# Roman-HLIS-Cosmology-PIT/romanimpreprocess

Measured on AMD Instinct MI355X. Metric: SCA ramps/sec (4096x4096x8grp full L1->L2 chain), higher is better.
Workload: dtype f32

## Files before the change

include/romanhip.h:

```cpp
#ifndef ROMANHIP_H
#define ROMANHIP_H

#include <stdint.h>

#ifdef __cplusplus
extern "C" {
#endif

#define RIP_VERSION 100
#define RIP_TIMING_BUILD_FLAG 1000000
#define RIP_MAX_GROUPS 64
#define RIP_CHANNEL_WIDTH 128

typedef struct rip_ctx rip_ctx;

typedef enum { RIP_OK = 0, RIP_EINVAL = -1, RIP_ENOMEM = -2, RIP_EHIP = -3, RIP_ESTATE = -4 } rip_status;
typedef enum { RIP_F32 = 0, RIP_F64 = 1, RIP_U16 = 2, RIP_F16 = 3 } rip_dtype;
typedef enum { RIP_HOST = 0, RIP_DEVICE = 1 } rip_location;
typedef enum { RIP_INPUTS_STREAM_ORDERED = 0, RIP_INPUTS_COMPLETE = 1 } rip_inputs_ready;

enum {
    RIP_STAGE_REFPIX = 1 << 0,
    RIP_STAGE_BIAS = 1 << 1,
    RIP_STAGE_LIN = 1 << 2,
// ... 174 lines not shown

int rip_stage_noise_1f(rip_ctx *ctx, int rows, int width, int nframes, const double *normals, uint64_t seed,
                       uint32_t stream_id, float *out);

int rip_stage_poisson_resample(rip_ctx *ctx, const float *skylevel, const void *gain, int gain_dtype, size_t n,
                               double frame_time, int ngrp, const int32_t *group_first, const int32_t *group_count,
                               const float *weights, const uint8_t *has_weights, const int8_t *endslice,
                               const double *samples, int nsamp, uint64_t seed, uint32_t layer, float *diff);


int rip_stats_l1_diff(rip_ctx *ctx, const uint16_t *cube, int ngrp, int ny, int nx, int ga, int gb, float *out);

int rip_stats_l2_pack(rip_ctx *ctx, const float *slope, const float *err_read, const float *err_poisson,
                      const uint32_t *pixeldq, int ny, int nx, int nb, const uint8_t grow[32], float *image, float *err,
                      uint8_t *good);

int rip_stats_reduce(rip_ctx *ctx, int nseeds, const float *diffs, const float *images, const float *errs, const uint8_t *good,
                     const float *ideal, int y0, int nrows, int ny, int nx, int nb, int alias_err, float *out);

int rip_profile_enable(rip_ctx *ctx, int on);
int rip_profile_read(rip_ctx *ctx, double out_ms[4], int *ncalls);

int rip_set_option(rip_ctx *ctx, const char *name, int value);
int rip_set_option_f64(rip_ctx *ctx, const char *name, double value);
int rip_get_option(rip_ctx *ctx, const char *name, int *value);
int rip_get_option_f64(rip_ctx *ctx, const char *name, double *value);
int rip_reset_options(rip_ctx *ctx);
int rip_option_info(int index, const char **name, int *def, int *lo, int *hi);

int rip_last_chain_form(rip_ctx *ctx);
int rip_last_chain_first_group(rip_ctx *ctx);
int rip_last_chain_bias_stream(rip_ctx *ctx);
int rip_last_prepass_gate(rip_ctx *ctx, int *giveups);

int rip_chain_form_for(int lin_nplanes, int ngroups, int ipc_dtype, int gain_dtype);

int rip_chain_geometry_for(int lin_nplanes, int ngroups, int ipc_dtype, int gain_dtype, int ny, int nx, int ncu, int reserve,
                           int quad_ok, int out[8]);
int rip_last_chain_geometry(rip_ctx *ctx, int out[8]);

int rip_stage_pearson(rip_ctx *ctx, size_t n, const double *I, double tilnu21, double tilnu31, double tilnu41, uint64_t seed,
                      uint32_t stream, double *draws, int32_t *types, double *params);

typedef struct rip_synth_cal {
    int32_t ny, nx, nb;
    int32_t channelwidth;
    int32_t nplanes;
    int32_t gain_dtype;
    int32_t ipc_dtype;
    int32_t amp33_valid;
    const void *gain;
    const float *read_noise;
    const float *resetnoise;
    const float *dark_slope;
    const float *dark;
    const float *lin_coefs;
    const float *smin, *smax;
    const void *ipc4d;
    const float *biascorr;
    double tbias;
    const float *amp33_med, *amp33_std;
    double m_pink, ru_pink;
    double u_pink, c_pink;
} rip_synth_cal;

int rip_synth_apportion(rip_ctx *ctx, const float *counts, int nya, int nxa, int poisson, int nreads, const double *t_reads,
// ... 83 lines not shown
```

romanimpreprocess_amd/_native.py:

```python

import contextlib
import ctypes as C
import os

import numpy as np

from . import _header

_HERE = os.path.dirname(os.path.abspath(__file__))
LIB_PATH = os.environ.get("ROMANHIP_LIB") or os.path.join(_HERE, "libromanhip.so")

with open(os.path.join(os.path.dirname(_HERE), "include", "romanhip.h")) as _f:
    HEADER = _header.parse(_f.read())
PROTOTYPES = HEADER.prototypes

globals().update(HEADER.constants)
globals().update({k[4:]: v for k, v in HEADER.constants.items() if k.startswith(("RIP_STAGE_", "RIP_BIAS_"))})

CaldirDesc = HEADER.structs["rip_caldir_desc"]
PlanDesc = HEADER.structs["rip_plan_desc"]
RampDesc = HEADER.structs["rip_ramp_desc"]
Outputs = HEADER.structs["rip_outputs"]
SynthCal = HEADER.structs["rip_synth_cal"]
CrParams = HEADER.structs["rip_cr_params"]
# ... 202 lines not shown
    def get_option_f64(self, name):
        v = C.c_double()
        self.call("rip_get_option_f64", name, C.byref(v))
        return v.value

    def reset_options(self):
        self.call("rip_reset_options")

    @contextlib.contextmanager
    def options(self, **values):
        calls = {name: ((self.get_option_f64, self.set_option_f64) if isinstance(v, float) else (self.get_option, self.set_option))
                 for name, v in values.items()}
        old = []
        try:
            for name, v in values.items():
                get, set_ = calls[name]
                before = get(name)
                set_(name, v)
                old.append((set_, name, before))
            yield self
        finally:
            for set_, name, before in reversed(old):
                set_(name, before)

    def last_chain_form(self):
        return self.call("rip_last_chain_form")

    def last_chain_first_group(self):
        return self.call("rip_last_chain_first_group")

    def last_prepass_gate(self):
        n = C.c_int(0)
        return self.call("rip_last_prepass_gate", C.byref(n)), n.value

    def caldir_first_group_safe(self, slot):
        return self.call("rip_caldir_first_group_safe", slot) == 1

    def caldir_bias_state(self, slot):
        return self.call("rip_caldir_bias_state", slot)

    def last_chain_bias_stream(self):
        return self.call("rip_last_chain_bias_stream")

    def last_chain_geometry(self):
        out = (C.c_int * 8)()
        self.call("rip_last_chain_geometry", out)
        return dict(zip(GEOMETRY_FIELDS, out))

    def profile(self, on=True):
        self.call("rip_profile_enable", bool(on))

    def profile_read(self):
        ms = (C.c_double * 4)()
        n = C.c_int(0)
        self.call("rip_profile_read", ms, C.byref(n))
        return list(ms), n.value

    @property
    def stream(self):
        return self.call("rip_stream")

    def upload_caldir(self, slot, cal, nborder=4, refout_slope=None):
        d = CaldirDesc()
        keep = []

        def P(a, dt):
# ... 76 lines not shown
```

romanimpreprocess_amd/csrc/api.hip:

```cpp
#include <limits.h>
#include <math.h>
#include <stdarg.h>
#include <stdio.h>
#include <string.h>

#include "rip_host.h"

static std::string g_create_error;

int rip_fail(rip_ctx *ctx, int code, const char *fmt, ...) {
    char buf[512];
    va_list ap;
    va_start(ap, fmt);
    vsnprintf(buf, sizeof buf, fmt, ap);
    va_end(ap);
    if (ctx)
        ctx->err = buf;
    else
        g_create_error = buf;
    return code;
}

void *rip_ws(rip_ctx *ctx, RipWs slot, size_t bytes) {
    if (ctx->ws_bytes[slot] >= bytes && ctx->ws[slot]) return ctx->ws[slot];
// ... 151 lines not shown
    if (ctx->stream2) RIP_HIP(ctx, hipStreamSynchronize(ctx->stream2));
    RIP_HIP(ctx, hipStreamSynchronize(ctx->stream));
    return RIP_OK;
}

void *rip_stream(rip_ctx *ctx) { return (void *)ctx->stream; }

void *rip_host_alloc(rip_ctx *ctx, size_t bytes) {
    void *p = nullptr;
    if (hipSetDevice(ctx->device) != hipSuccess || hipHostMalloc(&p, bytes ? bytes : 1, hipHostMallocDefault) != hipSuccess) {
        (void)rip_fail(ctx, RIP_ENOMEM, "rip_host_alloc: %zu bytes of page-locked memory", bytes);
        return nullptr;
    }
    return p;
}
void rip_host_free(rip_ctx *ctx, void *p) {
    (void)ctx;
    if (p) (void)hipHostFree(p);
}

int rip_option_info(int index, const char **name, int *def, int *lo, int *hi) {
    if (index < 0 || index >= (int)(sizeof k_options / sizeof k_options[0])) return 0;
    const RipOption &o = k_options[index];
    const auto as_int = [](double v) { return v <= INT_MIN ? INT_MIN : v >= INT_MAX ? INT_MAX : (int)v; };
    if (name) *name = o.name;
    if (def) *def = as_int(o.def);
    if (lo) *lo = as_int(o.lo);
    if (hi) *hi = as_int(o.hi);
    return o.f64 ? 2 : 1;
}

int rip_reset_options(rip_ctx *ctx) {
    for (const RipOption &o : k_options) store_option(ctx, o, o.def);
    return RIP_OK;
}

int rip_set_option(rip_ctx *ctx, const char *name, int value) { return set_option(ctx, name, false, value); }
int rip_set_option_f64(rip_ctx *ctx, const char *name, double value) { return set_option(ctx, name, true, value); }

int rip_get_option(rip_ctx *ctx, const char *name, int *value) {
    const RipOption *o = find_option(ctx, name, false);
    if (o) *value = ctx->*o->i;
    return o ? RIP_OK : RIP_EINVAL;
}
int rip_get_option_f64(rip_ctx *ctx, const char *name, double *value) {
    const RipOption *o = find_option(ctx, name, true);
    if (o) *value = ctx->*o->f64;
    return o ? RIP_OK : RIP_EINVAL;
}

int rip_chain_stamps(rip_ctx *ctx, double out[9]) {
    const size_t n = 4096 * 9;
    if (!ctx->chain_dbg_buf) {
        RIP_HIP(ctx, hipMalloc((void **)&ctx->chain_dbg_buf, n * 8));
        RIP_HIP(ctx, hipMemset(ctx->chain_dbg_buf, 0, n * 8));
        for (int i = 0; i < 9; ++i) out[i] = 0;
        return RIP_OK;
    }
    RIP_HIP(ctx, hipStreamSynchronize(ctx->stream));
    std::vector<unsigned long long> h(n);
    RIP_HIP(ctx, hipMemcpy(h.data(), ctx->chain_dbg_buf, n * 8, hipMemcpyDeviceToHost));
    for (int i = 0; i < 9; ++i) out[i] = 0;
    for (size_t k = 0; k < n; ++k) out[k % 9] += (double)h[k];
    RIP_HIP(ctx, hipMemset(ctx->chain_dbg_buf, 0, n * 8));
    return RIP_OK;
}
// ... 84 lines not shown
```

romanimpreprocess_amd/csrc/calibrate.hip:

```cpp
#include <string.h>

#include <cmath>

#include "rip_host.h"

size_t rip_host_ramp_bytes(const rip_ramp_desc &in, int ny, int nx) {
    const size_t G = in.ngrp, npix = (size_t)ny * nx;
    return al256(G * npix * (in.data_dtype == RIP_U16 ? 2 : 4)) + al256(G * ny * RIP_CW * 2) + al256(G * npix) + al256(npix * 4) +
           al256(npix * 8) + al256(G * (nx / RIP_CW) * 16) + al256(npix * 2) + al256((size_t)ny * RIP_CW * 2);
}

int rip_check_reference_read(rip_ctx *ctx, const rip_ramp_desc &in, const char *who) {
    if (!rip_ramp_is_encoded(in)) return RIP_OK;
    if (in.location == RIP_DEVICE)
        return rip_fail(ctx, RIP_EINVAL, "%s: reference_read / reference_amp33 come with host ramps only (a device caller decodes its arrays with "
                        "rip_stage_decode_reference_read and calibrates them as usual)", who);
    if (in.reference_read && in.data_dtype != RIP_U16) return rip_fail(ctx, RIP_EINVAL, "%s: reference_read needs u16 data", who);
    if (in.reference_amp33 && !in.amp33) return rip_fail(ctx, RIP_EINVAL, "%s: reference_amp33 without amp33", who);
    if (in.data_encoding_offset > (1 << 30) || in.data_encoding_offset < -(1 << 30))
        return rip_fail(ctx, RIP_EINVAL, "%s: data_encoding_offset %d (|offset| <= 2^30 supported)", who, (int)in.data_encoding_offset);
    return RIP_OK;
}

int rip_upload_host_ramp(rip_ctx *ctx, const rip_ramp_desc &in, int ny, int nx, char *w, hipStream_t st, rip_ramp_desc *dev,
// ... 287 lines not shown
        } else {
            ca.bias = c.dark_data;
            ca.bias_records = 0;
        }
        ca.planes = c.slab;
        ca.do_not_flag_first = plan->h.do_not_flag_first;
        ca.kern = c.ipc;
        ca.finish = (stages & (RIP_STAGE_DARK | RIP_STAGE_FLAT)) ? 1 : 0;
        if (stages & RIP_STAGE_DARK) {
            ca.dark_rate = 1;
            ca.dark_dq = c.has_dark_dq ? c.dark_dq : nullptr;
        }
        ca.flat = flat;
        ca.slope = o.slope;
        ca.err_read = o.err_read;
        ca.err_poisson = o.err_poisson;
        ca.pdq_out = o.pixeldq;
        ca.gdq_out = o.groupdq;
        float *cube = nullptr;
        if (out->cube) {
            cube = host ? (float *)rip_ws(ctx, RIP_WS_CUBE_B, (size_t)G * npix * 4) : out->cube;
            if (!cube) return RIP_ENOMEM;
            ca.cube_out = cube;
        }
        ca.ny = ny;
        ca.nx = nx;
        ca.nb = c.nb;
        ca.ngrp = G;
        ca.dense = plan->d_dense;
        ca.merged_dq = c.merged_plane[((flat ? 1 : 0) | ((stages & RIP_STAGE_DARK) ? 2 : 0))];
        ca.dbg = ctx->chain_dbg;
        ca.dbg_buf = ctx->chain_dbg_buf;
        ca.wg_counter = ctx->prepass_gate > 0 ? ctx->gate_words : nullptr;
        const int rc = rip_launch_chain(ctx, plan, ca, c.lin_nplanes, c.ipc_dtype, skip0);
        if (rc == 1 && skip0) return rip_fail(ctx, RIP_ESTATE, "calibrate: the fused kernel declined a launch planned without group 0");
        if (rc == 1) return RIP_OK;
        if (rc) return rc;
        ran_fused = true;
        cur = cube;
        for (int i = 0; i < 3; ++i) mark(ctx, ctx->stream);
        return RIP_OK;
    }

    int stage_kernels() {
        int rc;
        pdq_mid = d.pixeldq;
        if (do_ref || do_bias || do_lin || in->data_dtype != RIP_F32) {
            float *cubeA = (float *)rip_ws(ctx, RIP_WS_CUBE_A, (size_t)G * npix * 4 + npix * 4);
            if (!cubeA) return RIP_ENOMEM;
            uint32_t *pdq_ws = (uint32_t *)(cubeA + (size_t)G * npix);
            LinArgs la;
            memset(&la, 0, sizeof la);
            la.data = d.data;
            la.data_dtype = in->data_dtype;
            la.phi = cubeA;
            la.gdq = d.groupdq;
            la.gdq_is_attempt = 0;
            la.pdq_in = d.pixeldq;
            la.pdq_out = do_lin ? pdq_ws : nullptr;
            if (do_ref) {
                la.dark_data = c.dark_data;
                la.rowcorr = rowcorr;
                la.lines = lines;
            }
            if (do_bias) la.bias = c.bias + (size_t)(c.ngrp_bias - G) * npix;
            if (do_lin) {
// ... 112 lines not shown
```

romanimpreprocess_amd/csrc/chain2_kernel.h:

```cpp
#pragma once
#include "chain_common.h"
#include "chain2_form.h"

#if (defined(C2_DBG) || defined(CH_STAMP)) && !defined(RIP_TIMING_BUILD)
#error "C2_DBG / CH_STAMP are timing experiments: build them with -DRIP_TIMING_BUILD"
#endif
#ifdef CH_STAMP
#define C2_DRAIN()                                \
    if (a.dbg & 2048) {                           \
        __builtin_amdgcn_s_waitcnt(0);            \
    }
#else
#define C2_DRAIN()
#endif
#define C2_SYNC() __syncthreads()

__device__ __forceinline__ unsigned c2_opaque(unsigned x) {
    asm volatile("" : "+v"(x));
    return x;
}

__device__ __forceinline__ __amdgpu_buffer_rsrc_t c2_rsrc(const void *p, int records = -1) {
    return __builtin_amdgcn_make_buffer_rsrc(const_cast<void *>(p), 0, records, 0x00020000);
}
// ... 605 lines not shown
                            }
                            O12[(p0 * 3 + so) * COLS + col] = o1v;
                        }
                    }
                }
                if (GP * CO_STEP < NCO) fetch_coefs(kb2, r + 4, GP * CO_STEP, NCO, rr);
            }
            CH_T(5)
            CH_T(6)
            C2_SYNC();
            CH_T(7)
        }
    } else {
        f2 xnext[GP];
#pragma unroll
        for (int p0 = 0; p0 < GP; ++p0) xnext[p0] = f2{0.0f, 0.0f};
        const RipVariant v0 = rip_load_variant(vars, 0);
        const RipFitConst fc0 = rip_fit_const(h);
        constexpr int start = START;
        float gain_next = 1.0f;
        uint32_t dq_next = 0, qw_next[QW];
#pragma unroll
        for (int i = 0; i < QW; ++i) qw_next[i] = 0;
        int o0_r = (R0 - 5 + 3000) % 3;
        uint32_t qb_next[F::wring ? 1 : G];
#pragma unroll
        for (int g = 0; g < (F::wring ? 1 : G); ++g) qb_next[g] = 0;
        f2 kn[5];
        double kn_d[9];
#pragma unroll
        for (int i = 0; i < 5; ++i) kn[i] = f2{0.0f, 0.0f};
#pragma unroll
        for (int k = 0; k < 9; ++k) kn_d[k] = 0.0;
        for (int r = R0 - 5; r <= R0 + rows_wg; ++r, o0_r = (o0_r == 2) ? 0 : o0_r + 1) {
            const bool emit = (r >= R0) && (r < R1) && col_ok && (wcol >= 2 || c < 2) && (wcol < wl - 2 || c >= nx - 2);
            const RIP_K C2KernArgs *kf = c2_args(kargs);
            const unsigned rc_ = (unsigned)min(max(r, R0), yhi);
            const unsigned pe = rc_ * (unsigned)nx + cc1;
            const __amdgpu_buffer_rsrc_t rpl = c2_rsrc(kf->a.planes);
            const unsigned t_row = rc_ * row4;
            const unsigned t_ld = (dbg & 256) ? 0u : t_row;
            const float e_read = c2_ld_f32<SA>(rpl, cc4, (unsigned)(NP + 5) * pl4 + t_ld);
            const float e_gain = gain_next;
            const size_t t_row4 = (size_t)t_row;
            const size_t pe_row = (size_t)(rc_ * (unsigned)nx);
            const float e_dark = c2_ld_f32<SA>(rpl, cc4, (unsigned)(NP + 6) * pl4 + t_ld);
            const uint32_t e_pdq = c2_ld_u32<SA>(c2_rsrc(kf->a.pdq), cc4, t_ld);
            const float e_flat_raw = c2_ld_f32<SA>(c2_rsrc(kf->a.flat ? (const void *)kf->a.flat : (const void *)kf->a.planes), cc4, t_ld);
            const float e_flat = kf->a.flat ? e_flat_raw : 1.0f;
            float d[GE];
            f2 dpair[GP];
            uint32_t qw[QW];
#pragma unroll
            for (int i = 0; i < QW; ++i) qw[i] = 0;
            uint32_t lin_dq = 0;
            RipFitState fs;
            const bool act = emit && col_act && r >= ay0 && r < ay1;
            CH_T(0)
            C2_DRAIN()
            CH_T(1)
            f2 kF[5];
            double kFd[9];
            kF[4].y = 0.0f;
            if constexpr (KFIT) {
#pragma unroll
                for (int k = 0; k < 9; ++k) kFd[k] = kn_d[k];
#pragma unroll
                for (int i = 0; i < 5; ++i) kF[i] = kn[i];
            }
            if (emit) {
                if constexpr (KRN > 0) {
                    const int ks = r & 1;
                    if constexpr (K64) {
#pragma unroll
                        for (int k = 0; k < KRN; ++k) kFd[k] = KRd[(ks * KRN + k) * COLS + col];
                    } else {
#pragma unroll
                        for (int i = 0; i < 4; ++i) kF[i] = KR2[(ks * 4 + i) * COLS + col];
                        kF[4].x = KR1[ks * COLS + col];
                    }
                }
                const unsigned vF = k_valid(r);
#pragma unroll
                for (int i = 0; i < QW; ++i) qw[i] = qw_next[i];
                if constexpr (!F::wring) {
#pragma unroll
                    for (int i = 0; i < QW; ++i) qw[i] = 0;
#pragma unroll
                    for (int g = 0; g < G; ++g) qw[g / 4] |= (qb_next[g] & 0xffu) << (8 * (g & 3));
// ... 74 lines not shown
#pragma unroll
                            for (int b = 0; b < NBG; ++b) {
                                const f2 *ob = O12 + (p0 + b) * 3 * COLS;
                                om[b] = ob + om_ * COLS, o0[b] = ob + o0_ * COLS, op[b] = ob + op_ * COLS;
                            }
                            f2 f[NBG], oc[NBG];
                            if (all)
                                fwd_rows_batch<NBG, true>(om, o0, op, col, kF, vF, f, oc);
                            else
                                fwd_rows_batch<NBG, false>(om, o0, op, col, kF, vF, f, oc);
                            f2 o2[NBG];
#pragma unroll
                            for (int b = 0; b < NBG; ++b) o2[b] = (oc[b] + xc[b]) - f[b];
                            if (fastdiv) {
#pragma unroll
                                for (int b = 0; b < NBG; ++b) val[b] = div_rcp2(o2[b], e_gain, rgain);
                            } else {
#pragma unroll
                                for (int b = 0; b < NBG; ++b) val[b] = f2{o2[b].x / e_gain, o2[b].y / e_gain};
                            }
                        }
#pragma unroll
                        for (int b = 0; b < NBG; ++b) {
                            d[2 * (p0 + b)] = val[b].x;
                            d[2 * (p0 + b) + 1] = val[b].y;
                            dpair[p0 + b] = val[b];
                        }
                    }
                }
                if constexpr (GE > G) d[G] = 0.0f, dpair[GP - 1].y = 0.0f;
                if constexpr (SKIP0) d[0] = 0.0f, dpair[0].x = 0.0f;
                const bool unsat = ((qw[(G - 1) / 4] >> (8 * ((G - 1) & 3))) & DQ_SATURATED) == 0;
                if (!(dbg & 4))
                    fit_full_pk_a<G, rip_full_valid<G, START>(), SKIP0>(dpair, fc0, v0, kf->a.dense, e_gain, e_read, unsat && act, kf->guard, fs);
            }
            CH_T(2)
            C2_SYNC();
            CH_T(3)
            const RIP_K C2KernArgs *kg = c2_args(kargs);
            CH_T(4)
            C2_DRAIN()
            CH_T(5)
            float s = 0.0f, er = 0.0f, ep = 0.0f;
            uint32_t jmask = 0, pdq = 0;
            auto part_fb = [&]() {
                if constexpr (!SKIP0) {
                    if (kg->a.cube_out) {
#pragma unroll
                        for (int g = 0; g < G; ++g) kg->a.cube_out[(unsigned)g * npix + pe] = d[g];
                    }
                }
                uint32_t qor = 0;
#pragma unroll
                for (int i = 0; i < QW; ++i) qor |= qw[i];
                const bool anysat = (qor & 0x02020202u) != 0u;
                const bool unsat = ((qw[(G - 1) / 4] >> (8 * ((G - 1) & 3))) & DQ_SATURATED) == 0;
                if (dbg & 4) {
                    s = d[0], er = e_read, ep = e_gain;
                } else {
                    fit_full_pk_b<G>(dpair, kg->h, fc0, kg->a.dense, kg->kvals + v0.k_ofs, kg->diffs + v0.diff_ofs, unsat && act,
                                     fs, jmask);
                    s = fs.s, er = fs.er, ep = fs.ep;
                    if (__any(anysat)) {
                        uint32_t qe[G];
#pragma unroll
                        for (int g = 0; g < G; ++g) qe[g] = (qw[g / 4] >> (8 * (g & 3))) & 0xffu;
                        trunc_layers<G, G - 1, GE, SKIP0>(d, qe, kg->h, kg->vars, kg->kvals, kg->diffs, e_gain, e_read, act, kg->guard, s, er,
                                                          ep, jmask);
// ... 39 lines not shown
                part_finish();
            }
            {
                const int sn = (o0_r == 2) ? 0 : o0_r + 1;
#pragma unroll
                for (int p0 = 0; p0 < GP; ++p0) xnext[p0] = X2[(p0 * XR + sn) * COLS + col];
                dq_next = DQ[sn * COLS + col];
                if constexpr (F::wring) {
#pragma unroll
                    for (int i = 0; i < QW; ++i) qw_next[i] = QS[(sn * QW + i) * COLS + col];
                    gain_next = GN[sn * COLS + col];
                } else {
                    const unsigned yl = (unsigned)min(max((dbg & 1024) ? R0 : r + 1, ylo), yhi);
                    const __amdgpu_buffer_rsrc_t rq = c2_rsrc(kg->a.gdq);
                    unsigned o1 = yl * (row4 >> 2);
#pragma unroll
                    for (int g = 0; g < G; ++g) {
                        qb_next[g] = c2_ld_u8(rq, cc1, o1);
                        o1 += npix;
                    }
                    gain_next = c2_ld_f32(c2_rsrc(kg->a.planes), cc4, (unsigned)(NP + 4) * pl4 + yl * row4);
                }
            }
            if constexpr (KFIT) {
                if constexpr (K64)
                    (void)load_k(kg->a.kern, (dbg & 1024) ? R0 : r + 1, true, kn_d, C2Int<KRN>{});
                else
                    (void)load_k(kg->a.kern, (dbg & 1024) ? R0 : r + 1, true, kn, C2Int<0>{});
            }
            CH_T(6)
            C2_SYNC();
            CH_T(7)
        }
    }
#ifdef CH_STAMP
    if ((tid & 63) == 0 && a.dbg_buf) {
        unsigned long long *o = a.dbg_buf + ((size_t)blockIdx.x * (F::threads / 64) + (tid >> 6)) * 9;
        for (int i = 0; i < 9; ++i) o[i] += st_[i];
    }
#endif
}

template <int NP, int G, int START, typename KT, bool SKIP0 = false, bool BIAS = true>
static int launch_chain2_s(rip_ctx *ctx, const RipPlan *plan, const ChainArgs &a) {
    using F = C2Form<G + (G & 1), sizeof(KT) == 8>;
    const size_t lds = F::lds_bytes;
    if (a.nb < 2) return 1;
    ChainArgs ag = a;
    const long grid = c2_form_geometry<F>(ag, ctx->ncu, ctx->chain_reserve, ctx->chain_quad, ctx->last_geo);
    static bool lds_set[64] = {};
    if (lds > 48 * 1024 && !lds_set[ctx->device & 63]) {
        RIP_HIP(ctx, hipFuncSetAttribute(reinterpret_cast<const void *>(chain2_kernel<NP, G, START, KT, SKIP0, BIAS>),
                                         hipFuncAttributeMaxDynamicSharedMemorySize, (int)lds));
        lds_set[ctx->device & 63] = true;
    }
    hipLaunchKernelGGL((chain2_kernel<NP, G, START, KT, SKIP0, BIAS>), dim3((unsigned)grid), dim3(F::threads), lds, ctx->stream, ag,
                       reinterpret_cast<const RipPlanHeader *>(plan->dev), plan->d_variants, plan->d_k, plan->d_diffs,
                       ctx->guard_band);
    RIP_HIP(ctx, hipGetLastError());
    if (ag.wg_counter) ctx->gate_total += (uint32_t)grid, ctx->gate_armed = true;
    return RIP_OK;
}

template <int NP, int G, typename KT, bool BIAS>
static int launch_chain2_b(rip_ctx *ctx, const RipPlan *plan, const ChainArgs &a, bool skip0) {
    if (plan->h.start == 0 && plan->dense.valid == rip_full_valid<G, 0>())
// ... 29 lines not shown
```

romanimpreprocess_amd/csrc/device_rampfit.h:

```cpp
#pragma once
#include "rip_common.h"

#define RIP_K __attribute__((address_space(4)))
template <typename T>
__device__ __forceinline__ const RIP_K T *rip_k(const T *p) {
    return (const RIP_K T *)p;
}
#define KLD(x) (*rip_k(&(x)))
__device__ __forceinline__ RipVariant rip_load_variant(const RipVariant *vars, int i) {
    RipVariant v;
    v.g = KLD(vars[i].g);
    v.ndiff = KLD(vars[i].ndiff);
    v.diff_ofs = KLD(vars[i].diff_ofs);
    v.k_ofs = KLD(vars[i].k_ofs);
    v.coef = KLD(vars[i].coef);
    v.rfac = KLD(vars[i].rfac);
    return v;
}

__device__ __forceinline__ float log_f32(float x) {
    return (float)log((double)x);
}

__device__ __forceinline__ float hypot_f32(float a, float b) {
// ... 376 lines not shown

struct RipFitConst {
    float ia, ib;
    float sa32;
    float slope_th;
    float inv_ia;
};
__device__ __forceinline__ RipFitConst rip_fit_const(const RipPlanHeader *h) {
    RipFitConst c;
    c.ia = KLD(h->ia);
    c.ib = KLD(h->ib);
    c.sa32 = (float)KLD(h->sa);
    c.slope_th = (float)(KLD(h->dsb) / KLD(h->loglen));
    c.inv_ia = 1.0f / c.ia;
    return c;
}

__device__ __forceinline__ void rip_load_pair(RipDensePair &r, const RipDense *dn, int ps) {
#pragma unroll
    for (int e = 0; e < 2; ++e) {
        r.inv_dt[e] = KLD(dn->pairs[ps].inv_dt[e]);
        r.A[e] = KLD(dn->pairs[ps].A[e]);
        r.B[e] = KLD(dn->pairs[ps].B[e]);
        r.k1[e] = KLD(dn->pairs[ps].k1[e]);
        r.k2[e] = KLD(dn->pairs[ps].k2[e]);
    }
}

template <int G, int START>
constexpr uint32_t rip_full_valid() {
    return rip_full_valid_of(G, START);
}

struct RipFitState {
    float s, er, ep;
    float dv, s2, xc;
    uint32_t jfast, unsure;
    bool live;
};

template <int G, uint32_t VALID = 0u, bool SKIP0 = false>
__device__ __forceinline__ void fit_full_pk_a(const rf2 (&dA)[(G + 1) / 2], const RipFitConst fc, const RipVariant v,
                                              const RipDense *__restrict__ dn, float gain, float rn, bool flag, double guard,
                                              RipFitState &st) {
    constexpr int GP = (G + 1) / 2;
    constexpr int NS = 2 * GP;
    float k2[G];
#pragma unroll
    for (int t = 0; t < G; ++t) k2[t] = KLD(dn->K2[t]);
    const uint32_t valid = VALID ? VALID : KLD(dn->valid);
    RipDensePair tab[2];
    rip_load_pair(tab[0], dn, 0);
    const float d1 = dA[0].y;
    const rf2 d11 = {d1, d1};
    float s = 0.0f;
#pragma unroll
    for (int p = 0; p < GP; ++p) {
        const rf2 diff = dA[p] - d11;
        if constexpr (SKIP0) {
            if (p == 0) {
                const float prod = k2[1] * diff.y;
                s = s + prod;
                continue;
            }
        }
        if constexpr (G & 1) {
            if (2 * p + 1 >= G) {
                const float prod = k2[2 * p] * diff.x;
                s = s + prod;
                continue;
            }
        }
        const rf2 kk = {k2[2 * p], k2[2 * p + 1]};
        const rf2 prod = kk * diff;
        s = s + prod.x;
        s = s + prod.y;
    }
    float dv;
    rip_slope_errors<float, true>(s, gain, rn, v, dv, st.er, st.ep);
    st.s = s;
    st.dv = dv;
    st.s2 = rn * rn;
    st.jfast = 0;
    st.unsure = 0;
    st.xc = 0.0f;
    st.live = __any(flag);
    if (!st.live) return;

    const float xc = clip2<float>(s, fc.ia, fc.ib);
    st.xc = xc;
    const bool need_log = xc != fc.ia;
    float lx = 0.0f;
    if (__any(need_log)) lx = need_log ? __logf(xc * fc.inv_ia) : 0.0f;
    const float slope_th = fc.slope_th;
    const float sth32 = fc.sa32 + slope_th * lx;
    const float band0 = 2e-6f * fabsf(sth32) + 4.5e-6f * fabsf(slope_th) + 1e-30f;
    const float s2 = st.s2;
    const float s8 = fabsf(s) * 8.1e-7f;
    const float thp = sth32 + band0, thm = sth32 - band0;
    const float rsmax = __frsqrt_rn(KLD(dn->amin) * s2) * 1.000001f;
    const bool pass = fmaf(s8, rsmax, band0) <= 0.5f * sth32;
    const bool lane_exact = !(guard < 1e300) || !pass;
    const float tmax = s8 * rsmax;
    const float hp = thp + tmax, lm = thm - tmax;
    uint32_t jfast = 0, unsure_mask = 0;
    rf2 dB[GP];
#pragma unroll
    for (int p = 0; p < GP; ++p) dB[p] = rf2{dA[p].y, (p + 1 < GP) ? dA[p + 1].x : 0.0f};
#pragma unroll
    for (int ps = 0; ps < NS; ++ps) {
        if (ps + 1 < NS) rip_load_pair(tab[(ps + 1) & 1], dn, ps + 1);
        const int ip = ps / 2, di = (ps & 1) + 1;
        const uint32_t vbits = (valid >> (2 * ps)) & 3u;
        if (vbits == 0) continue;
        const rf2 hi = (di == 1) ? dB[ip] : ((ip + 1 < GP) ? dA[ip + 1] : rf2{0.0f, 0.0f});
        const rf2 lo = dA[ip];
        const RipDensePair &r = tab[ps & 1];
        const rf2 num = hi - lo;
        const rf2 q = num * rf2{r.inv_dt[0], r.inv_dt[1]};
        const rf2 delta = q - rf2{s, s};
        const rf2 as2 = rf2{r.A[0], r.A[1]} * s2;
        const rf2 var = __builtin_elementwise_fma(rf2{r.B[0], r.B[1]}, rf2{dv, dv}, as2);
        const rf2 rs = {__frsqrt_rn(var.x), __frsqrt_rn(var.y)};
        const rf2 sm = delta * rs;
        const rf2 hiT = rf2{hp, hp} * rf2{r.k1[0], r.k1[1]};
        const rf2 loT = rf2{lm, lm} * rf2{r.k2[0], r.k2[1]};
#pragma unroll
        for (int e = 0; e < 2; ++e) {
            if (!((vbits >> e) & 1u)) continue;
            const float sme = e ? sm.y : sm.x;
            const bool hit = sme > (e ? hiT.y : hiT.x);
            const bool nohit = sme < (e ? loT.y : loT.x);
            if (hit) jfast |= 1u << (2 * ps + e);
            if (lane_exact || !(hit || nohit)) unsure_mask |= 1u << (2 * ps + e);
        }
    }
    st.jfast = jfast;
    st.unsure = unsure_mask;
}

template <int G>
// ... 107 lines not shown
```

romanimpreprocess_amd/csrc/plan.hip:

```cpp
#include <string.h>

#include <cmath>
#include <memory>

#include "rip_host.h"

static std::vector<float> variant_weights(const rip_plan_desc *d, int v, int g, int start) {
    std::vector<float> K(g, 0.0f);
    if (v == 0) {
        for (int i = 0; i < g; ++i) K[i] = d->K[i];
    } else {
        K[g - 1] = 1.0f / (d->tbar[g - 1] - d->tbar[start]);
        K[start] = -K[g - 1];
    }
    return K;
}

extern "C" {

int rip_plan_desc_first_weight_zero(const rip_plan_desc *d) {
    if (!d || !d->exclude_first || d->ngrp < 3 || d->ngrp > RIP_MAX_GROUPS) return 0;
    const int G = d->ngrp, nvar = 1 + (G - 4 > 0 ? G - 4 : 0);
    for (int v = 0; v < nvar; ++v)
        if (variant_weights(d, v, v == 0 ? G : G - v, 1)[0] != 0.0f) return 0;
// ... 73 lines not shown
    const size_t o_d = o_k + al(p->kvals.size() * sizeof(float));
    const size_t o_dense = o_d + al(p->diffs.size() * sizeof(RipDiff));
    p->bytes = o_dense + al(sizeof(RipDense));
    {
        RipDense &dn = p->dense;
        memset(&dn, 0, sizeof dn);
        for (int i = 0; i < G; ++i) dn.K2[i] = d->K[i];
        const RipVariant &v0 = p->variants[0];
        double amin = 1e301;
        for (int k = 0; k < v0.ndiff; ++k) {
            const RipDiff &df = p->diffs[v0.diff_ofs + k];
            const int i = df.i, di = df.j - df.i, ps = 2 * (i / 2) + (di - 1), e = i & 1;
            if (G <= 16) dn.valid |= 1u << (2 * ps + e);
            dn.kidx[2 * ps + e] = k;
            dn.pairs[ps].inv_dt[e] = df.inv_dt;
            dn.pairs[ps].A[e] = df.A;
            dn.pairs[ps].B[e] = df.B;
            const double r = (double)df.relerr + 4.1e-7;
            if (r < 9.9e-3) {
                dn.pairs[ps].k1[e] = std::nextafter((float)((1.0 / (1.0 - r)) * (1.0 + 4e-7)), INFINITY);
            } else {
                dn.pairs[ps].k1[e] = INFINITY;
            }
            amin = (df.B >= 0.0f) ? std::fmin(amin, (double)df.A) : 0.0;
        }
        dn.amin = (v0.ndiff > 0 && amin > 0.0 && amin < 1e300) ? (float)(amin * (1.0 - 1e-6)) : 0.0f;
        for (int ps = 0; ps < RIP_MAX_GROUPS; ++ps)
            for (int e = 0; e < 2; ++e) {
                const int bit = 2 * ps + e;
                const bool used = bit < 32 && ((dn.valid >> bit) & 1u);
                if (!used) dn.pairs[ps].A[e] = 1.0f;
                dn.pairs[ps].k2[e] = 2.0f - dn.pairs[ps].k1[e];
            }
    }
    p->k0_zero = rip_plan_desc_first_weight_zero(d) == 1;
    std::vector<char> img(p->bytes, 0);
    memcpy(img.data(), &h, sizeof h);
    memcpy(img.data() + o_var, p->variants.data(), p->variants.size() * sizeof(RipVariant));
    memcpy(img.data() + o_k, p->kvals.data(), p->kvals.size() * sizeof(float));
    if (!p->diffs.empty()) memcpy(img.data() + o_d, p->diffs.data(), p->diffs.size() * sizeof(RipDiff));
    memcpy(img.data() + o_dense, &p->dense, sizeof(RipDense));
    hipError_t e = hipMalloc(&p->dev, p->bytes);
    if (e == hipSuccess) e = hipMemcpy(p->dev, img.data(), p->bytes, hipMemcpyHostToDevice);
    if (e != hipSuccess) return rip_fail(ctx, RIP_EHIP, "plan upload: %s", hipGetErrorString(e));
    p->d_variants = reinterpret_cast<const RipVariant *>((char *)p->dev + o_var);
    p->d_k = reinterpret_cast<const float *>((char *)p->dev + o_k);
    p->d_diffs = reinterpret_cast<const RipDiff *>((char *)p->dev + o_d);
    p->d_dense = reinterpret_cast<const RipDense *>((char *)p->dev + o_dense);
    int id = -1;
    for (size_t i = 0; i < ctx->plans.size(); ++i)
        if (!ctx->plans[i]) {
            id = (int)i;
            break;
        }
    if (id < 0) {
        ctx->plans.push_back(nullptr);
        id = (int)ctx->plans.size() - 1;
    }
    ctx->plans[id] = p.release();
    *plan_id = id;
    return RIP_OK;
}

int rip_plan_destroy(rip_ctx *ctx, int id) {
    if (id < 0 || id >= (int)ctx->plans.size() || !ctx->plans[id]) return rip_fail(ctx, RIP_EINVAL, "plan %d does not exist", id);
    RIP_HIP(ctx, hipStreamSynchronize(ctx->stream));
// ... 15 lines not shown
```

romanimpreprocess_amd/csrc/rip_common.h:

```cpp
#pragma once

#include <hip/hip_runtime.h>
#include <stdint.h>

#include <string>
#include <map>
#include <vector>

#include "../../include/romanhip.h"

#define DQ_DO_NOT_USE 0x1u
#define DQ_SATURATED 0x2u
#define DQ_JUMP_DET 0x4u
#define DQ_NO_FLAT_FIELD (1u << 18)
#define DQ_NO_GAIN_VALUE (1u << 19)
#define DQ_NO_LIN_CORR (1u << 20)
#define DQ_REFERENCE_PIXEL (1u << 31)

#define RIP_CW RIP_CHANNEL_WIDTH

struct RipDiff {
    int32_t i, j;
    float dt;
    float A, B;
    float inv_dt;
    float relerr;
    float pad_[1];
};

struct RipVariant {
    int32_t g;
    int32_t ndiff, diff_ofs, k_ofs;
    float coef, rfac;
};

struct RipPlanHeader {
    int32_t ngrp, start, nvariants, do_not_flag_first;
    double sa, dsb;
    double loglen;
    float ia, ib;
    float tbar[RIP_MAX_GROUPS], tau[RIP_MAX_GROUPS], nreads[RIP_MAX_GROUPS];
};

struct RipDensePair {
    float inv_dt[2], A[2], B[2];
    float k1[2];
    float k2[2];
};
struct RipDense {
    uint32_t valid;
    int32_t kidx[2 * RIP_MAX_GROUPS];
    float amin;
    float K2[RIP_MAX_GROUPS];
    RipDensePair pairs[RIP_MAX_GROUPS];
};

constexpr uint32_t rip_full_valid_of(int G, int start) {
    uint32_t m = 0;
    for (int i = start; i < G - 1; ++i) {
        const int dimax = (i == G - 2 || G - 1 - start == 2) ? 1 : 2;
        for (int di = 1; di <= dimax; ++di) m |= 1u << (2 * (2 * (i / 2) + (di - 1)) + (i & 1));
    }
    return m;
}

struct RipPlan {
    RipPlanHeader h;
    std::vector<RipVariant> variants;
    std::vector<float> kvals;
    std::vector<RipDiff> diffs;
    void *dev = nullptr;
    const RipVariant *d_variants = nullptr;
    const float *d_k = nullptr;
    const RipDiff *d_diffs = nullptr;
    const RipDense *d_dense = nullptr;
    RipDense dense;
    size_t bytes = 0;
    bool k0_zero = false;
};

struct RipCal {
    bool valid = false;
    int ny = 0, nx = 0, nb = 0;
    int ngrp_dark = 0, ngrp_bias = 0, lin_nplanes = 0;
    int gain_dtype = RIP_F32, ipc_dtype = RIP_F32;
    bool has_amp33 = false, has_ipc = false, has_flat = false, has_bias = false, has_dark_dq = false;
    double refout_slope = 0.0;
// ... 13 lines not shown
    float *bias = nullptr;
    bool bias_dropped = false;
    float *sat_thr = nullptr;
    uint32_t *sat_dq = nullptr;
    float *slab = nullptr;
    int merged_plane[4] = {3, -1, -1, -1};
    bool first_group_safe = false;
    bool has_inf = false;
    size_t bytes = 0;
};

enum RipWs {
    RIP_WS_CUBE_A = 0,
    RIP_WS_CUBE_B = 1,
    RIP_WS_STAGING = 2,
    RIP_WS_TABLES = 3,
    RIP_WS_REFPIX = 4,
    RIP_WS_IPC_X = 5,
    RIP_WS_IPC_A = 6,
    RIP_WS_RESULTS = 7,
    RIP_WS_SATFLAG = 8,
    RIP_WS_EXCEED = 9,
    RIP_WS_SHARE_TAB = 10,
    RIP_WS_SYNTH_START = 11,
    RIP_WS_FRAMES = 12,
    RIP_WS_SEL_HIST = 13,
    RIP_WS_R1_ZERO = 14,
    RIP_WS_R1_SCRATCH = 15,
    RIP_WS_DEFER = 16,
    RIP_WS_CR_TAB = 17,
    RIP_WS_COUNT
};

enum { RIP_GATE_COUNTER = 0, RIP_GATE_GIVEUPS = 32, RIP_GATE_STATE = 33, RIP_GATE_WORDS = 64 };

struct rip_ctx {
    int device = 0;
    int ncu = 0;
    std::string err;
    std::vector<RipCal> cals;
    std::vector<RipPlan *> plans;

    hipStream_t stream = nullptr;
    hipStream_t stream2 = nullptr;
    hipEvent_t ev_tab[2] = {nullptr, nullptr}, ev_done[2] = {nullptr, nullptr};
    bool ev_done_valid[2] = {false, false};
    int parity = 0;
    bool stream_dirty = false;
    hipEvent_t ev_in = nullptr;
    hipEvent_t ev_pre = nullptr;
    hipStream_t pre_stream = nullptr;
    bool ev_pre_valid = false;
    uint32_t *gate_words = nullptr;
    uint32_t gate_total = 0;
    bool gate_armed = false;
    bool in_batch = false;
    int prepass_gate;
    int last_gate = 0;
    int wall_khz = 100000;

    void *ws[RIP_WS_COUNT] = {};
    size_t ws_bytes[RIP_WS_COUNT] = {};

    bool can_overlap = false;
    int overlap_mode;
    int use_fused;
    int use_chain2;
    double guard_band;
    int chain_quad;
    int skip_first;
    int chain_reserve;
    int prepass_form;

    int last_form = 0;
    int last_first_group = 0;
    int last_bias_stream = 0;
    int last_geo[8] = {};
    int chain_dbg;
    unsigned long long *chain_dbg_buf = nullptr;
    void *prepass_stamps = nullptr;
    bool prof = false;
    std::vector<hipEvent_t> prof_events;

    hipStream_t stream3 = nullptr;
    void *batch_buf[4] = {nullptr, nullptr, nullptr, nullptr};
    size_t batch_bytes[4] = {0, 0, 0, 0};
    int batch_completed = 0;

    unsigned long long *refread_dev = nullptr, *refread_host = nullptr;
    int refread_cap = 0;

    void *pink_plan = nullptr, *pink_z = nullptr, *pink_s = nullptr, *pink_tab = nullptr;
    bool pink_own = false;
    int pink_form;
    hipEvent_t ev_pink = nullptr;
    hipStream_t pink_stream = nullptr;
    bool ev_pink_valid = false;
    size_t pink_L = 0;
    int pink_chunk = 0;

    hipEvent_t ev_frames = nullptr, ev_fill = nullptr, ev_ahead = nullptr;
    bool frames_pending = false, ev_fill_valid = false;
    uint64_t frames_seed = 0;
    int frames_geom[3] = {0, 0, 0};
    std::vector<double> share_tab;
    rip_cr_params cr_tab_key = {};
    bool cr_tab_valid = false;
};
// ... 47 lines not shown
    int do_not_flag_first;
    int ny, nx, nb, ngrp;
};
int rip_launch_lin(rip_ctx *ctx, const LinArgs &a);

struct ChainArgs {
    const void *data;
    int data_u16;
    const uint8_t *gdq;
    const uint32_t *pdq;
    const float *dark_data;
    const double *rowcorr, *lines;
    const double *rowcorr_t;
    const float *bias;
    const float *planes;
    int do_not_flag_first;
    int bias_records;
    const void *kern;
    int finish;
    int dark_rate;
    const uint32_t *dark_dq;
    const float *flat;
    float *slope, *err_read, *err_poisson;
    uint32_t *pdq_out;
    uint8_t *gdq_out;
    float *cube_out;
    const RipDense *dense;
    unsigned long long *dbg_buf;
    int merged_dq;
    int dbg;
    int ny, nx, nb, ngrp;
    int geo_nr, geo_rows, geo_nq, geo_rows_q;
    uint32_t *wg_counter;
};
#define RIP_CHAIN_G_PART0(X) X(5) X(6) X(7) X(8)
#define RIP_CHAIN_G_PART1(X) X(9) X(10) X(11) X(12)
#define RIP_CHAIN_G_PART2(X) X(13) X(14) X(15) X(16)
#define RIP_CHAIN_G_ALL(X) RIP_CHAIN_G_PART0(X) RIP_CHAIN_G_PART1(X) RIP_CHAIN_G_PART2(X)
bool rip_chain_supported(const rip_ctx *ctx, int nplanes, int G, int k_dtype, int gain_dtype);
bool rip_chain_fills_lds(int G, int k_dtype);
int rip_launch_chain(rip_ctx *ctx, const RipPlan *plan, const ChainArgs &a, int nplanes, int k_dtype, bool skip0 = false);
bool rip_chain_may_skip_first(const rip_ctx *ctx, const RipPlan *plan, int nplanes, int G, int k_dtype, int gain_dtype, int merged_dq,
                              int nb);

struct IpcArgs {
    const float *in;
    float *out;
    const void *kern;
    const void *gain;
    int k_dtype, g_dtype;
    int ny, nx, nb, ngrp;
};
int rip_launch_ipc_cube(rip_ctx *ctx, const IpcArgs &a);
int rip_launch_ipc_image(rip_ctx *ctx, int reverse, int order, const void *img, int img_dtype, int ny, int nx,
                         const void *kern , int k_dtype, const void *gain, int g_dtype, void *out);

struct RefpixArgs {
    const void *data;
    int data_dtype;
    const float *dark_data;
    const uint16_t *amp33;
    const float *amp33_med;
    double slope;
    const double *lines_override;
    double *rowcorr;
    double *rowcorr_t;
// ... 36 lines not shown
```

Measured before the change: 1298.

## Add conservative jump screen to skip full pairwise ramp fit for clean wavefronts

Adds a cheap precomputed per-difference bound check (inv_dt, A2, B2 tables built at plan time with a safety margin) that runs before the full pairwise jump-detection loop in the fused ramp fit. If every active lane in a wavefront passes the bound, the fit marks the wave settled and returns early, avoiding the expensive pair-table loads and comparisons. Optional counters record settled and live wavefronts for diagnostics. It costs an extra screening pass and table loads for wavefronts that fail, and relies on the margin being truly conservative so results stay identical.

```diff
diff --git a/include/romanhip.h b/include/romanhip.h
--- a/include/romanhip.h
+++ b/include/romanhip.h
@@ -230,6 +230,8 @@
 int rip_last_chain_first_group(rip_ctx *ctx);
 int rip_last_chain_bias_stream(rip_ctx *ctx);
 int rip_last_prepass_gate(rip_ctx *ctx, int *giveups);
+int rip_jump_screen(rip_ctx *ctx, int mode);
+int rip_last_chain_screened(rip_ctx *ctx, unsigned *settled, unsigned *live);
 
 int rip_chain_form_for(int lin_nplanes, int ngroups, int ipc_dtype, int gain_dtype);
 
diff --git a/romanimpreprocess_amd/_native.py b/romanimpreprocess_amd/_native.py
--- a/romanimpreprocess_amd/_native.py
+++ b/romanimpreprocess_amd/_native.py
@@ -258,6 +258,22 @@
     def last_prepass_gate(self):
         n = C.c_int(0)
         return self.call("rip_last_prepass_gate", C.byref(n)), n.value
+
+    def jump_screen(self, mode=-1):
+        return self.call("rip_jump_screen", mode)
+
+    @contextlib.contextmanager
+    def jump_screen_mode(self, mode):
+        before = self.jump_screen(mode)
+        try:
+            yield self
+        finally:
+            self.jump_screen(before)
+
+    def last_chain_screened(self):
+        settled, live = C.c_uint(0), C.c_uint(0)
+        self.call("rip_last_chain_screened", C.byref(settled), C.byref(live))
+        return settled.value, live.value
 
     def caldir_first_group_safe(self, slot):
         return self.call("rip_caldir_first_group_safe", slot) == 1
diff --git a/romanimpreprocess_amd/csrc/api.hip b/romanimpreprocess_amd/csrc/api.hip
--- a/romanimpreprocess_amd/csrc/api.hip
+++ b/romanimpreprocess_amd/csrc/api.hip
@@ -207,6 +207,25 @@
 
 int rip_reset_options(rip_ctx *ctx) {
     for (const RipOption &o : k_options) store_option(ctx, o, o.def);
+    ctx->jump_screen = 1;
+    return RIP_OK;
+}
+
+int rip_jump_screen(rip_ctx *ctx, int mode) {
+    if (!ctx) return RIP_EINVAL;
+    if (mode > 3) return rip_fail(ctx, RIP_EINVAL, "jump_screen mode must be in 0 .. 3 (negative: query)");
+    const int before = ctx->jump_screen;
+    if (mode >= 0) ctx->jump_screen = mode;
+    return before;
+}
+int rip_last_chain_screened(rip_ctx *ctx, unsigned *settled, unsigned *live) {
+    if (!ctx || !settled || !live) return RIP_EINVAL;
+    *settled = *live = 0;
+    if (ctx->last_form != 2 || !ctx->last_screen_counted) return RIP_OK;
+    RIP_HIP(ctx, hipStreamSynchronize(ctx->stream));
+    uint32_t w[2] = {0, 0};
+    RIP_HIP(ctx, hipMemcpy(w, ctx->gate_words + RIP_GATE_SCREEN, sizeof w, hipMemcpyDeviceToHost));
+    *settled = w[0], *live = w[1];
     return RIP_OK;
 }
 
diff --git a/romanimpreprocess_amd/csrc/calibrate.hip b/romanimpreprocess_amd/csrc/calibrate.hip
--- a/romanimpreprocess_amd/csrc/calibrate.hip
+++ b/romanimpreprocess_amd/csrc/calibrate.hip
@@ -343,6 +343,12 @@
         ca.dbg = ctx->chain_dbg;
         ca.dbg_buf = ctx->chain_dbg_buf;
         ca.wg_counter = ctx->prepass_gate > 0 ? ctx->gate_words : nullptr;
+        ca.jump_screen = ctx->jump_screen & 1;
+        ctx->last_screen_counted = (ctx->jump_screen & 2) && ctx->gate_words;
+        if (ctx->last_screen_counted) {
+            ca.screen_count = ctx->gate_words + RIP_GATE_SCREEN;
+            RIP_HIP(ctx, hipMemsetAsync(ca.screen_count, 0, 2 * sizeof(uint32_t), ctx->stream));
+        }
         const int rc = rip_launch_chain(ctx, plan, ca, c.lin_nplanes, c.ipc_dtype, skip0);
         if (rc == 1 && skip0) return rip_fail(ctx, RIP_ESTATE, "calibrate: the fused kernel declined a launch planned without group 0");
         if (rc == 1) return RIP_OK;
diff --git a/romanimpreprocess_amd/csrc/chain2_kernel.h b/romanimpreprocess_amd/csrc/chain2_kernel.h
--- a/romanimpreprocess_amd/csrc/chain2_kernel.h
+++ b/romanimpreprocess_amd/csrc/chain2_kernel.h
@@ -661,6 +661,7 @@
         for (int i = 0; i < 5; ++i) kn[i] = f2{0.0f, 0.0f};
 #pragma unroll
         for (int k = 0; k < 9; ++k) kn_d[k] = 0.0;
+        uint32_t n_live = 0, n_settled = 0;
         for (int r = R0 - 5; r <= R0 + rows_wg; ++r, o0_r = (o0_r == 2) ? 0 : o0_r + 1) {
             const bool emit = (r >= R0) && (r < R1) && col_ok && (wcol >= 2 || c < 2) && (wcol < wl - 2 || c >= nx - 2);
             const RIP_K C2KernArgs *kf = c2_args(kargs);
@@ -684,6 +685,7 @@
             for (int i = 0; i < QW; ++i) qw[i] = 0;
             uint32_t lin_dq = 0;
             RipFitState fs;
+            fs.live = fs.settled = false;
             const bool act = emit && col_act && r >= ay0 && r < ay1;
             CH_T(0)
             C2_DRAIN()
@@ -824,8 +826,11 @@
                 if constexpr (SKIP0) d[0] = 0.0f, dpair[0].x = 0.0f;
                 const bool unsat = ((qw[(G - 1) / 4] >> (8 * ((G - 1) & 3))) & DQ_SATURATED) == 0;
                 if (!(dbg & 4))
-                    fit_full_pk_a<G, rip_full_valid<G, START>(), SKIP0>(dpair, fc0, v0, kf->a.dense, e_gain, e_read, unsat && act, kf->guard, fs);
-            }
+                    fit_full_pk_a<G, rip_full_valid<G, START>(), SKIP0>(dpair, fc0, v0, kf->a.dense, e_gain, e_read, unsat && act, kf->guard,
+                                                                        kf->a.jump_screen != 0, fs);
+            }
+            n_live += __any(fs.live) ? 1u : 0u;
+            n_settled += __any(fs.settled) ? 1u : 0u;
             CH_T(2)
             C2_SYNC();
             CH_T(3)
@@ -931,6 +936,11 @@
             C2_SYNC();
             CH_T(7)
         }
+        uint32_t *sc = c2_args(kargs)->a.screen_count;
+        if (sc && __builtin_amdgcn_mbcnt_hi(~0u, __builtin_amdgcn_mbcnt_lo(~0u, 0u)) == 0u) {
+            __hip_atomic_fetch_add(sc, n_settled, __ATOMIC_RELAXED, __HIP_MEMORY_SCOPE_AGENT);
+            __hip_atomic_fetch_add(sc + 1, n_live, __ATOMIC_RELAXED, __HIP_MEMORY_SCOPE_AGENT);
+        }
     }
 #ifdef CH_STAMP
     if ((tid & 63) == 0 && a.dbg_buf) {
diff --git a/romanimpreprocess_amd/csrc/device_rampfit.h b/romanimpreprocess_amd/csrc/device_rampfit.h
--- a/romanimpreprocess_amd/csrc/device_rampfit.h
+++ b/romanimpreprocess_amd/csrc/device_rampfit.h
@@ -432,17 +432,45 @@
     return rip_full_valid_of(G, START);
 }
 
+struct RipScreenWalk {
+    int8_t i[32], j[32];
+};
+constexpr RipScreenWalk rip_screen_walk(uint32_t valid) {
+    RipScreenWalk w = {};
+    int k = 0;
+    for (int bit = 0; bit < 32; ++bit)
+        if ((valid >> bit) & 1u) {
+            const int ps = bit / 2, e = bit & 1;
+            w.i[k] = (int8_t)(2 * (ps / 2) + e);
+            w.j[k] = (int8_t)(w.i[k] + (ps & 1) + 1);
+            ++k;
+        }
+    return w;
+}
+#define RIP_SCREEN_CHUNK 4
+template <int NSCR>
+__device__ __forceinline__ void rip_load_screen(RipScreenDiff (&r)[RIP_SCREEN_CHUNK], const RipDense *dn, int c) {
+#pragma unroll
+    for (int e = 0; e < RIP_SCREEN_CHUNK; ++e)
+        if (c * RIP_SCREEN_CHUNK + e < NSCR) {
+            r[e].inv_dt = KLD(dn->scr[c * RIP_SCREEN_CHUNK + e].inv_dt);
+            r[e].A2 = KLD(dn->scr[c * RIP_SCREEN_CHUNK + e].A2);
+            r[e].B2 = KLD(dn->scr[c * RIP_SCREEN_CHUNK + e].B2);
+        }
+}
+
 struct RipFitState {
     float s, er, ep;
     float dv, s2, xc;
     uint32_t jfast, unsure;
     bool live;
+    bool settled;
 };
 
 template <int G, uint32_t VALID = 0u, bool SKIP0 = false>
 __device__ __forceinline__ void fit_full_pk_a(const rf2 (&dA)[(G + 1) / 2], const RipFitConst fc, const RipVariant v,
                                               const RipDense *__restrict__ dn, float gain, float rn, bool flag, double guard,
-                                              RipFitState &st) {
+                                              bool screen, RipFitState &st) {
     constexpr int GP = (G + 1) / 2;
     constexpr int NS = 2 * GP;
     float k2[G];
@@ -450,7 +478,14 @@
     for (int t = 0; t < G; ++t) k2[t] = KLD(dn->K2[t]);
     const uint32_t valid = VALID ? VALID : KLD(dn->valid);
     RipDensePair tab[2];
-    rip_load_pair(tab[0], dn, 0);
+    screen = VALID != 0u && screen && guard < 1e300;
+    constexpr int NSCR = __builtin_popcount(VALID);
+    constexpr RipScreenWalk walk = rip_screen_walk(VALID);
+    RipScreenDiff scr[2][RIP_SCREEN_CHUNK];
+    if (screen)
+        rip_load_screen<NSCR>(scr[0], dn, 0);
+    else
+        rip_load_pair(tab[0], dn, 0);
     const float d1 = dA[0].y;
     const rf2 d11 = {d1, d1};
     float s = 0.0f;
@@ -485,6 +520,7 @@
     st.unsure = 0;
     st.xc = 0.0f;
     st.live = __any(flag);
+    st.settled = false;
     if (!st.live) return;
 
     const float xc = clip2<float>(s, fc.ia, fc.ib);
@@ -507,6 +543,35 @@
     rf2 dB[GP];
 #pragma unroll
     for (int p = 0; p < GP; ++p) dB[p] = rf2{dA[p].y, (p + 1 < GP) ? dA[p + 1].x : 0.0f};
+    if (screen) {
+        const float lm2 = lm * lm;
+        const float u = lm2 * s2, w = lm2 * dv;
+        uint64_t clean = __ballot(!lane_exact && lm <= 1e3f && u >= 1e-16f && u <= 1e30f && w <= 1e30f);
+#pragma unroll
+        for (int c = 0; c * RIP_SCREEN_CHUNK < NSCR; ++c) {
+            if ((c + 1) * RIP_SCREEN_CHUNK < NSCR) rip_load_screen<NSCR>(scr[(c + 1) & 1], dn, c + 1);
+#pragma unroll
+            for (int e = 0; e < RIP_SCREEN_CHUNK; ++e) {
+                const int k = c * RIP_SCREEN_CHUNK + e;
+                if (k >= NSCR) continue;
+                const int i = walk.i[k], j = walk.j[k];
+                const float hi = (j & 1) ? dA[j / 2].y : dA[j / 2].x, lo = (i & 1) ? dA[i / 2].y : dA[i / 2].x;
+                const RipScreenDiff r = scr[c & 1][e];
+                const float nnum = lo - hi;
+                const float nq = nnum * r.inv_dt;
+                const float ndelta = nq + s;
+                const float bound = fmaf(r.B2, w, r.A2 * u);
+                const float np = ndelta * fabsf(ndelta);
+                clean &= __builtin_amdgcn_fcmpf(-np, bound, 4);
+            }
+            __builtin_amdgcn_sched_barrier(0);
+        }
+        if ((__ballot(flag) & ~clean) == 0) {
+            st.settled = true;
+            return;
+        }
+        rip_load_pair(tab[0], dn, 0);
+    }
 #pragma unroll
     for (int ps = 0; ps < NS; ++ps) {
         if (ps + 1 < NS) rip_load_pair(tab[(ps + 1) & 1], dn, ps + 1);
diff --git a/romanimpreprocess_amd/csrc/plan.hip b/romanimpreprocess_amd/csrc/plan.hip
--- a/romanimpreprocess_amd/csrc/plan.hip
+++ b/romanimpreprocess_amd/csrc/plan.hip
@@ -129,6 +129,23 @@
                 if (!used) dn.pairs[ps].A[e] = 1.0f;
                 dn.pairs[ps].k2[e] = 2.0f - dn.pairs[ps].k1[e];
             }
+        const auto toward_zero = [](double x) {
+            const float f = (float)x;
+            return ((double)f > x) ? std::nextafter(f, 0.0f) : f;
+        };
+        for (int k = 0; k < RIP_SCREEN_DIFFS; ++k) dn.scr[k].inv_dt = dn.scr[k].A2 = dn.scr[k].B2 = NAN;
+        int nscr = 0;
+        for (int bit = 0; bit < 32; ++bit) {
+            if (!((dn.valid >> bit) & 1u)) continue;
+            const RipDensePair &pr = dn.pairs[bit / 2];
+            const int e = bit & 1;
+            RipScreenDiff &sd = dn.scr[nscr++];
+            sd.inv_dt = pr.inv_dt[e];
+            const double kk = (double)pr.k2[e] * (double)pr.k2[e] * (1.0 - RIP_SCREEN_MARGIN);
+            const double a2 = (double)pr.A[e] * kk, b2 = (double)pr.B[e] * kk;
+            if (pr.k2[e] > 0.0f && pr.k2[e] <= 1.0f && a2 >= 1e-12 && a2 <= 1e6 && b2 >= 0.0 && b2 <= 1e6)
+                sd.A2 = toward_zero(a2), sd.B2 = toward_zero(b2);
+        }
     }
     p->k0_zero = rip_plan_desc_first_weight_zero(d) == 1;
     std::vector<char> img(p->bytes, 0);
diff --git a/romanimpreprocess_amd/csrc/rip_common.h b/romanimpreprocess_amd/csrc/rip_common.h
--- a/romanimpreprocess_amd/csrc/rip_common.h
+++ b/romanimpreprocess_amd/csrc/rip_common.h
@@ -47,12 +47,18 @@
     float k1[2];
     float k2[2];
 };
+struct RipScreenDiff {
+    float inv_dt, A2, B2;
+};
+#define RIP_SCREEN_MARGIN (32.0 / 16777216.0)
+#define RIP_SCREEN_DIFFS 32
 struct RipDense {
     uint32_t valid;
     int32_t kidx[2 * RIP_MAX_GROUPS];
     float amin;
     float K2[RIP_MAX_GROUPS];
     RipDensePair pairs[RIP_MAX_GROUPS];
+    RipScreenDiff scr[RIP_SCREEN_DIFFS] __attribute__((aligned(16)));
 };
 
 constexpr uint32_t rip_full_valid_of(int G, int start) {
@@ -132,7 +138,7 @@
     RIP_WS_COUNT
 };
 
-enum { RIP_GATE_COUNTER = 0, RIP_GATE_GIVEUPS = 32, RIP_GATE_STATE = 33, RIP_GATE_WORDS = 64 };
+enum { RIP_GATE_COUNTER = 0, RIP_GATE_GIVEUPS = 32, RIP_GATE_STATE = 33, RIP_GATE_SCREEN = 40, RIP_GATE_WORDS = 64 };
 
 struct rip_ctx {
     int device = 0;
@@ -174,6 +180,8 @@
 
     int last_form = 0;
     int last_first_group = 0;
+    int jump_screen = 1;
+    bool last_screen_counted = false;
     int last_bias_stream = 0;
     int last_geo[8] = {};
     int chain_dbg;
@@ -287,6 +295,8 @@
     int ny, nx, nb, ngrp;
     int geo_nr, geo_rows, geo_nq, geo_rows_q;
     uint32_t *wg_counter;
+    int jump_screen;
+    uint32_t *screen_count;
 };
 #define RIP_CHAIN_G_PART0(X) X(5) X(6) X(7) X(8)
 #define RIP_CHAIN_G_PART1(X) X(9) X(10) X(11) X(12)
```

New measurement: 1306 (median of 6 runs). No clear change (+0.6%).
